# roseDwayane/EyeGaze-Multimodal

Hardware: AMD Instinct MI355X
Metric: train samples/sec (gaze+EEG windows) (higher is better)
Workload: dtype bf16; 1 GPU; cfg3: BASELINE configs[2]/[3]: + bidirectional cross-stream attention fusion; batch_per_gpu=256, global_batch=256, C=8, T=1024, seq_len=65, d_model=256, layers=6, step=fwd(train,dropout)+bwd+allreduce+clip+AdamW, parallelism=dp1

## Files before the change

### eyegaze_multimodal_amd/csrc/heads.hip

```cpp
#include "common.h"

namespace {

template <typename T>
__global__ void rows_bcast_f32_kernel(const float* __restrict__ src, const float* __restrict__ pos, T* __restrict__ dst,
                                      int NB, int S, int D, int R, int off, int src_nb) {
  const int b = blockIdx.y, r = blockIdx.x;
  const float* s = src + ((size_t)(b % src_nb) * R + r) * D;
  T* d = dst + ((size_t)b * S + off + r) * D;
  for (int n = threadIdx.x; n < D; n += blockDim.x) {
    float v = s[n];
    if (pos) v += pos[(size_t)(off + r) * D + n];
    Elem<T>::st(d + n, v);
  }
}

template <typename T>
__global__ void rows_copy_kernel(T* __restrict__ seq, int S, int D, int R, int off, int b_src0, int b_dst0) {
  const int b = blockIdx.y, r = blockIdx.x;
  const T* s = seq + ((size_t)(b_src0 + b) * S + off + r) * D;
  T* d = seq + ((size_t)(b_dst0 + b) * S + off + r) * D;
  for (int n = threadIdx.x; n < D; n += blockDim.x) d[n] = s[n];
}

// ... 480 lines not shown
          float g4[4];
          load4((const T*)&gv[u], g4);
#pragma unroll
          for (int e = 0; e < 4; ++e) v[e] = g4[e] > 0.f ? v[e] * gate_scale : 0.f;
          store4(dst + row_off(dmap, b * R + (s - off)) + n, v);
        }
      }
    }
  };
  for (int i = 0; i < iters; i += 8) rows8(r + 16 * i, 16, min(8, iters - i));
  if (j == 0) {
    const int b0 = bl + 16 * iters;
    if (b0 < NB) rows8(b0, 4, (NB - b0 + 3) / 4);
  }
#pragma unroll
  for (int e = 0; e < 4; ++e) red[r][tx * 4 + e] = acc[e];
  __syncthreads();
  if (threadIdx.x < 64) {
    const int c = threadIdx.x;
    float a[4];
#pragma unroll
    for (int l = 0; l < 4; ++l) a[l] = (red[l][c] + red[l + 4][c]) + (red[l + 8][c] + red[l + 12][c]);
    const float t = a[0] + a[1] + a[2] + a[3];
    const int col = blockIdx.y * 64 + c;
    out[(size_t)s * D + col] = t;
    if (s == 0 && cls_out) cls_out[col] = t;
  }
}

constexpr int HD = 256;
constexpr int HK = 3 * HD;
constexpr int HP = HD + 8;

template <typename T, int NT, int KS>
__device__ __forceinline__ void head_mma(f32x4 (&acc)[NT], const T* xrow, const T* __restrict__ W, const int ldw, const int n0,
                                         const int lane) {
  typedef typename H16<T>::frag frag;
  const int l15 = lane & 15, g = lane >> 4;
  const T* wp = W + (size_t)(n0 + l15) * ldw + 8 * g;
  frag wf[KS][NT];
#pragma unroll
  for (int ks = 0; ks < KS; ++ks)
#pragma unroll
    for (int t = 0; t < NT; ++t) wf[ks][t] = *(const frag*)(wp + (size_t)16 * t * ldw + 32 * ks);
  __builtin_amdgcn_sched_barrier(0);
#pragma unroll
  for (int ks = 0; ks < KS; ++ks) {
    const frag xf = *(const frag*)(xrow + 32 * ks);
#pragma unroll
    for (int t = 0; t < NT; ++t) acc[t] = H16<T>::mfma(wf[ks][t], xf, acc[t]);
  }
}

template <typename T>
struct HeadsFwd {
  const T* comb; T* zf; T* hcl; const T* Wsf; const T* Wc0;
  const float* bsf; const float* bc0; const float* W3; const float* b3;
  const long long* labels; float* logits; float* sloss; float* loss; unsigned int* counter;
  const eg_step_state* st;
  int B, ncls;
  DropCfg d1;
};

constexpr int HKP = HK + 8;
template <typename T>
__global__ __launch_bounds__(512) void heads_fwd_kernel(HeadsFwd<T> p) {
  __shared__ __attribute__((aligned(16))) T xs[2][16][HKP];
  __shared__ __attribute__((aligned(16))) T hs[16][HP];
  __shared__ float red[256];
  __shared__ int last_s;
  const int tid = threadIdx.x, lane = tid & 63, wave = tid >> 6;
  const int l15 = lane & 15, g = lane >> 4;
  const int m0 = blockIdx.x * 16;
  const int m = m0 + l15;
  const int n0 = 32 * wave;
  for (int c = tid; c < 16 * (HK / 8); c += 512) {
    const int r = c / (HK / 8), ch = c % (HK / 8);
    const size_t row = (size_t)min(m0 + r, p.B - 1) * HK;
    *(u32x4*)&xs[0][r][ch * 8] = *(const u32x4*)(p.comb + row + ch * 8);
    if (ch >= HD / 8) *(u32x4*)&xs[1][r][ch * 8] = *(const u32x4*)(p.zf + row + ch * 8);
  }
  __syncthreads();

  f32x4 acc[2];
#pragma unroll
  for (int t = 0; t < 2; ++t) acc[t] = (f32x4){0.f, 0.f, 0.f, 0.f};
  head_mma<T, 2, HK / 32>(acc, &xs[0][l15][8 * g], p.Wsf, HK, n0, lane);
#pragma unroll
  for (int t = 0; t < 2; ++t) {
    const int n = n0 + 16 * t + 4 * g;
    float bv[4], v[4];
    load4(p.bsf + n, bv);
#pragma unroll
    for (int e = 0; e < 4; ++e) v[e] = acc[t][e] + bv[e];
    store4(&xs[1][l15][n], v);
    if (m < p.B) store4(p.zf + (size_t)m * HK + n, v);
    acc[t] = (f32x4){0.f, 0.f, 0.f, 0.f};
  }
  __syncthreads();
  head_mma<T, 2, HK / 32>(acc, &xs[1][l15][8 * g], p.Wc0, HK, n0, lane);
  uint32_t seed_lo = 0, seed_hi = 0;
  if (p.d1.thresh) {
    seed_lo = p.st->seed_lo;
    seed_hi = p.st->seed_hi;
  }
#pragma unroll
  for (int t = 0; t < 2; ++t) {
    const int n = n0 + 16 * t + 4 * g;
    float bv[4], v[4];
    load4(p.bc0 + n, bv);
#pragma unroll
    for (int e = 0; e < 4; ++e) v[e] = fmaxf(acc[t][e] + bv[e], 0.f);
    eg_dropout_run<4>(v, p.d1, seed_lo, seed_hi, (uint32_t)m * (uint32_t)HD + (uint32_t)n);
    store4(&hs[l15][n], v);
    if (m < p.B) store4(p.hcl + (size_t)m * HD + n, v);
  }
  __syncthreads();
#pragma unroll
  for (int i = 0; i < 2; ++i) {
    const int r = 2 * wave + i;
    if (m0 + r < p.B)
      classifier_ce_fwd_row<T>(&hs[r][0], p.W3, p.b3, p.labels, p.logits, p.sloss, m0 + r, HD, p.ncls, lane);
  }
  if (!p.labels) return;
  __threadfence();
  __syncthreads();
  if (tid == 0) last_s = atomicAdd(p.counter, 1u) == gridDim.x - 1;
  __syncthreads();
  if (!last_s || tid >= 256) return;
  __threadfence();
  block_mean256<true>(p.sloss, p.loss, p.B, red);
  if (tid == 0) *p.counter = 0u;
}

constexpr int TNP = 128 + 8;
template <typename T>
__device__ __forceinline__ void small_tn_tile(const T* __restrict__ dY, const int ldy, const T* __restrict__ X, const int ldx,
                                              float* __restrict__ dW, float* __restrict__ db, const int M, const int K,
                                              const int tile, char* smem) {
  typedef typename H16<T>::frag frag;
  T (*Yt)[TNP] = (T(*)[TNP])smem;
  T (*Xt)[TNP] = (T(*)[TNP])(smem + 64 * TNP * sizeof(T));
  const int tid = threadIdx.x, lane = tid & 63, wave = tid >> 6;
  const int l15 = lane & 15, g = lane >> 4;
  const int tiles_k = K / 64;
  const int n0 = (tile / tiles_k) * 64, k0 = (tile % tiles_k) * 64;
  const int nsplit = M > 128 ? 2 : 1;
  const int kw = wave & 3, t0 = (wave >> 2) * 2, t1 = blockDim.x == 512 ? t0 + 2 : 4;
  f32x4 acc[2][4];
#pragma unroll
  for (int sp = 0; sp < 2; ++sp)
#pragma unroll
    for (int t = 0; t < 4; ++t) acc[sp][t] = (f32x4){0.f, 0.f, 0.f, 0.f};
  float bsplit[2] = {0.f, 0.f};
  for (int sp = 0; sp < nsplit; ++sp) {
    if (sp) __syncthreads();
    for (int c = tid; c < 1024; c += blockDim.x) {
      const int row = c >> 3, ch = c & 7;
      const int m = 128 * sp + row;
      u32x4 y = {0u, 0u, 0u, 0u}, x = {0u, 0u, 0u, 0u};
      if (m < M) {
        y = *(const u32x4*)(dY + (size_t)m * ldy + n0 + ch * 8);
        x = *(const u32x4*)(X + (size_t)m * ldx + k0 + ch * 8);
      }
      const uint16_t* ye = (const uint16_t*)&y;
// ... 10 lines not shown
      const frag xf = *(const frag*)&Xt[16 * kw + l15][32 * ks + 8 * g];
#pragma unroll
      for (int t = 0; t < 4; ++t)
        if (t >= t0 && t < t1) {
          const frag yf = *(const frag*)&Yt[16 * t + l15][32 * ks + 8 * g];
          acc[sp][t] = H16<T>::mfma(xf, yf, acc[sp][t]);
        }
    }
    if (db && k0 == 0 && tid < 64) {
      float bh[2] = {0.f, 0.f};
      for (int sub = 0; sub < 4; ++sub)
#pragma unroll
        for (int half = 0; half < 2; ++half) {
          float cs = 0.f;
#pragma unroll
          for (int i = 0; i < 16; ++i) cs += H16<T>::ld(Yt[tid][32 * sub + 16 * half + i]);
          bh[half] += cs;
        }
      bsplit[sp] = bh[0] + bh[1];
    }
  }
#pragma unroll
  for (int t = 0; t < 4; ++t)
    if (t >= t0 && t < t1) {
      const int n = n0 + 16 * t + l15, k = k0 + 16 * kw + 4 * g;
      f32x4 o = acc[0][t];
      if (nsplit == 2) o += acc[1][t];
      *(f32x4*)(dW + (size_t)n * K + k) = o;
    }
  if (db && k0 == 0 && tid < 64) db[n0 + tid] = nsplit == 2 ? bsplit[0] + bsplit[1] : bsplit[0];
}
constexpr int TN_SMEM = 2 * 64 * TNP * 2;

template <typename T>
__global__ __launch_bounds__(256) void classifier_ce_bwd_fused_kernel(const T* __restrict__ h, const float* __restrict__ W,
                                                                      const float* __restrict__ logits,
                                                                      const long long* __restrict__ labels,
                                                                      const float* __restrict__ gloss,
                                                                      const float* __restrict__ glogits,
                                                                      float* __restrict__ dlogits, T* __restrict__ dh,
                                                                      float* __restrict__ dW, float* __restrict__ db, int B,
                                                                      int K, int ncls, int use_gate, float gate_scale, int nce) {
  __shared__ __attribute__((aligned(16))) T hts[256][64];
  __shared__ float dls[256][16];
  __shared__ float red[4][64], redb[4];
  const int lane = threadIdx.x & 63, bl = threadIdx.x >> 6;
  if ((int)blockIdx.x < nce) {
    const int b = blockIdx.x * 4 + bl;
    if (b < B) classifier_ce_bwd_row<T>(b, lane, h, W, logits, labels, gloss, glogits, dlogits, dh, B, K, ncls, use_gate, gate_scale);
    return;
  }
  const int kb = (blockIdx.x - nce) * 64, k = kb + lane;
  const bool wide = kb + 64 <= K && K % 8 == 0;
  for (int c = threadIdx.x; c < B * 8; c += 256) {
    const int b = c >> 3, ch = c & 7;
    if (wide) *(u32x4*)&hts[b][ch * 8] = *(const u32x4*)(h + (size_t)b * K + kb + ch * 8);
    else
      for (int e = 0; e < 8; ++e)
        if (kb + ch * 8 + e < K) hts[b][ch * 8 + e] = h[(size_t)b * K + kb + ch * 8 + e];
  }
  for (int b = threadIdx.x; b < B; b += 256) {
    float dl[16];
    classifier_dlogits_row(logits, labels, gloss, glogits, b, B, ncls, dl);
#pragma unroll
    for (int c = 0; c < 16; ++c) dls[b][c] = dl[c];
  }
  __syncthreads();
  float s[16], sb[16];
#pragma unroll
  for (int c = 0; c < 16; ++c) s[c] = sb[c] = 0.f;
  for (int b = bl; b < B; b += 4) {
    const float hv = H16<T>::ld(hts[b][lane]);
#pragma unroll
    for (int c = 0; c < 16; ++c)
      if (c < ncls) {
        const float dl = dls[b][c];
        if (k < K) s[c] = fmaf(dl, hv, s[c]);
        sb[c] += dl;
      }
  }
#pragma unroll
  for (int c = 0; c < 16; ++c)
    if (c < ncls) {
      red[bl][lane] = s[c];
      if (lane == 0) redb[bl] = sb[c];
      __syncthreads();
      if (bl == 0) {
        if (k < K) dW[(size_t)c * K + k] = red[0][lane] + red[1][lane] + red[2][lane] + red[3][lane];
        if (kb == 0 && lane == 0) db[c] = redb[0] + redb[1] + redb[2] + redb[3];
      }
      __syncthreads();
    }
}

template <typename T>
__global__ __launch_bounds__(512) void heads_bwd_chain_kernel(const T* __restrict__ dhcl, const T* __restrict__ c0T,
                                                              const T* __restrict__ sfT, const T* __restrict__ zf,
                                                              T* __restrict__ dzf, T* __restrict__ dcomb, float* __restrict__ dWc0,
                                                              float* __restrict__ dbc0, int B, int nrt) {
  __shared__ __attribute__((aligned(16))) char smem[TN_SMEM];
  if ((int)blockIdx.x >= nrt) {
    small_tn_tile<T>(dhcl, HD, zf, HK, dWc0, dbc0, B, HK, blockIdx.x - nrt, smem);
    return;
  }
  T (*xs)[16][HP] = (T(*)[16][HP])smem;
  const int tid = threadIdx.x, lane = tid & 63, wave = tid >> 6;
  const int l15 = lane & 15, g = lane >> 4;
  const int m0 = blockIdx.x * 16;
  const int m = m0 + l15;
  {
    const int r = tid >> 5, ch = tid & 31;
    *(u32x4*)&xs[0][r][ch * 8] = *(const u32x4*)(dhcl + (size_t)min(m0 + r, B - 1) * HD + ch * 8);
  }
  __syncthreads();
#pragma unroll 1
  for (int prod = 0; prod < 2; ++prod) {
    const T* W = prod ? sfT : c0T;
    T* out = prod ? dcomb : dzf;
    const int n0 = 96 * wave;
    f32x4 acc[6];
#pragma unroll
    for (int t = 0; t < 6; ++t) acc[t] = (f32x4){0.f, 0.f, 0.f, 0.f};
    head_mma<T, 6, HD / 32>(acc, &xs[prod][l15][8 * g], W, HD, n0, lane);
#pragma unroll
    for (int t = 0; t < 6; ++t) {
      const int n = n0 + 16 * t + 4 * g;
      float v[4] = {acc[t][0] + 0.f, acc[t][1] + 0.f, acc[t][2] + 0.f, acc[t][3] + 0.f};
      if (!prod && n < HD) store4(&xs[1][l15][n], v);
      if (m < B) store4(out + (size_t)m * HK + n, v);
    }
    __syncthreads();
  }
}

template <typename T>
__global__ __launch_bounds__(256) void heads_bwd_pool_kernel(const T* __restrict__ z, const T* __restrict__ dcomb,
                                                             const T* __restrict__ dzf, const float* __restrict__ gcls1,
                                                             const float* __restrict__ gcls2, const T* __restrict__ dibs_pool,
                                                             const float* __restrict__ gibs_pool, T* __restrict__ dz,
                                                             const T* __restrict__ comb, float* __restrict__ dWsf,
                                                             float* __restrict__ dbsf, int B, int S, int D, int off, int n_ibs,
                                                             int ibs_first) {
  __shared__ __attribute__((aligned(16))) char smem[TN_SMEM];
  if ((int)blockIdx.x >= B) {
    small_tn_tile<T>(dzf, HK, comb, HK, dWsf, dbsf, B, HK, blockIdx.x - B, smem);
    return;
  }
  pool_fuse_bwd_sample<T>(blockIdx.x, z, dcomb, dzf, gcls1, gcls2, dibs_pool, gibs_pool, dz, B, S, D, off, n_ibs, ibs_first);
}

}

extern "C" int eg_rows_bcast_f32(const float* src, const float* pos, void* seq, int NB, int S, int D, int R, int off,
                                 int src_nb, int dtype, void* stream) {
  if (eg_dtype_check("eg_rows_bcast_f32", dtype, true)) return 1;
  EG_CHECK(src && seq && NB > 0 && R > 0 && off >= 0 && off + R <= S && src_nb > 0, "eg_rows_bcast_f32: bad arguments");
  dim3 grid(R, NB);
  hipStream_t s = (hipStream_t)stream;
  eg_dispatch_dtype(dtype, [&](auto t) {
    using T = typename decltype(t)::type;
    hipLaunchKernelGGL(rows_bcast_f32_kernel<T>, grid, dim3(256), 0, s, src, pos, (T*)seq, NB, S, D, R, off, src_nb);
  });
  EG_LAUNCH_CHECK("rows_bcast_f32");
  return 0;
}
// ... 109 lines not shown
  EG_LAUNCH_CHECK("rows_gather_gate");
  return 0;
}

extern "C" int eg_token_grad_tail(const void* dseq, const void* gate, void* dst, eg_rowmap dmap, float* pos_grad,
                                  float* cls_grad, int NB, int S, int D, int R, int off, float gate_scale, int dtype,
                                  void* stream) {
  if (eg_dtype_check("eg_token_grad_tail", dtype, false)) return 1;
  EG_CHECK(dseq && gate && dst && pos_grad, "eg_token_grad_tail: null pointer");
  EG_CHECK(NB > 0 && S > 0 && R > 0 && off >= 0 && off + R <= S, "eg_token_grad_tail: bad shape NB=%d S=%d R=%d off=%d", NB, S, R, off);
  EG_CHECK(D > 0 && D % 64 == 0, "eg_token_grad_tail: D=%d must be a multiple of 64", D);
  EG_CHECK(dmap.row_stride % 4 == 0 && dmap.group_stride % 4 == 0, "eg_token_grad_tail: destination rows must be 8-B aligned");
  hipStream_t s = (hipStream_t)stream;
  dim3 grid(S, D / 64);
  eg_dispatch_16(dtype, [&](auto t) {
    using T = typename decltype(t)::type;
    hipLaunchKernelGGL(token_grad_tail_kernel<T>, grid, dim3(256), 0, s, (const T*)dseq, (const T*)gate, (T*)dst, to_rowmap(dmap), pos_grad,
                       cls_grad, NB, S, D, R, off, gate_scale);
  });
  EG_LAUNCH_CHECK("token_grad_tail");
  return 0;
}

template <typename T>
static void launch_heads_fwd(const void* comb, void* zf, void* hcl, const void* Wsf, const float* bsf, const void* Wc0,
                             const float* bc0, const float* W3, const float* b3, const int64_t* labels, float* logits,
                             float* sloss, float* loss, uint32_t* counter, int B, int ncls, float drop_p, uint32_t drop_site,
                             const eg_step_state* state, hipStream_t s) {
  HeadsFwd<T> p;
  p.comb = (const T*)comb; p.zf = (T*)zf; p.hcl = (T*)hcl; p.Wsf = (const T*)Wsf; p.Wc0 = (const T*)Wc0;
  p.bsf = bsf; p.bc0 = bc0; p.W3 = W3; p.b3 = b3;
  p.labels = (const long long*)labels; p.logits = logits; p.sloss = sloss; p.loss = loss; p.counter = counter;
  p.st = state; p.B = B; p.ncls = ncls; p.d1 = make_drop(drop_p, drop_site);
  hipLaunchKernelGGL(heads_fwd_kernel<T>, dim3((B + 15) / 16), dim3(512), 0, s, p);
}

extern "C" int eg_heads_fwd(const void* comb, void* zf, void* hcl, const void* Wsf, const float* bsf, const void* Wc0,
                            const float* bc0, const float* W3, const float* b3, const int64_t* labels, float* logits,
                            float* sample_loss, float* loss, uint32_t* counter, int B, int D, int ncls, float drop_p,
                            uint32_t drop_site, const eg_step_state* state, int dtype, void* stream) {
  if (eg_dtype_check("eg_heads_fwd", dtype, false)) return 1;
  EG_CHECK(comb && zf && hcl && Wsf && bsf && Wc0 && bc0 && W3 && b3 && logits, "eg_heads_fwd: null pointer");
  EG_CHECK(D == HD, "eg_heads_fwd: d_model=%d (the fused heads are built for 256)", D);
  EG_CHECK(B > 0 && ncls > 0 && ncls <= 16, "eg_heads_fwd: B=%d, ncls=%d must be in [1,16]", B, ncls);
  EG_CHECK(!labels || (sample_loss && loss && counter), "eg_heads_fwd: labels need sample_loss, loss and the launch counter");
  EG_CHECK(drop_p >= 0.f && drop_p < 1.f && (drop_p == 0.f || state), "eg_heads_fwd: dropout needs the step state");
  EG_CHECK(((uintptr_t)comb | (uintptr_t)zf | (uintptr_t)hcl | (uintptr_t)Wsf | (uintptr_t)Wc0 | (uintptr_t)bsf | (uintptr_t)bc0) % 16 == 0,
           "eg_heads_fwd: alignment");
  hipStream_t s = (hipStream_t)stream;
  eg_dispatch_16(dtype, [&](auto t) {
    launch_heads_fwd<typename decltype(t)::type>(comb, zf, hcl, Wsf, bsf, Wc0, bc0, W3, b3, labels, logits, sample_loss, loss, counter, B,
                                                 ncls, drop_p, drop_site, state, s);
  });
  EG_LAUNCH_CHECK("heads_fwd");
  return 0;
}

extern "C" int eg_classifier_ce_bwd_fused(const void* h, const float* W, const float* logits, const int64_t* labels,
                                          const float* gloss, const float* glogits, float* dlogits, void* dh, float* dW,
                                          float* db, int B, int K, int ncls, int use_gate, float gate_scale, int dtype,
                                          void* stream) {
  if (eg_dtype_check("eg_classifier_ce_bwd_fused", dtype, false)) return 1;
  EG_CHECK(h && W && logits && dlogits && dh && dW && db, "eg_classifier_ce_bwd_fused: null pointer");
  EG_CHECK(B > 0 && B <= 256 && K > 0 && ncls > 0 && ncls <= 16, "eg_classifier_ce_bwd_fused: bad shape B=%d (<= 256) K=%d ncls=%d", B, K, ncls);
  EG_CHECK((uintptr_t)h % 16 == 0, "eg_classifier_ce_bwd_fused: alignment");
  hipStream_t s = (hipStream_t)stream;
  const int nce = (B + 3) / 4;
  dim3 grid(nce + (K + 63) / 64);
  eg_dispatch_16(dtype, [&](auto t) {
    using T = typename decltype(t)::type;
    hipLaunchKernelGGL(classifier_ce_bwd_fused_kernel<T>, grid, dim3(256), 0, s, (const T*)h, W, logits, (const long long*)labels, gloss,
                       glogits, dlogits, (T*)dh, dW, db, B, K, ncls, use_gate, gate_scale, nce);
  });
  EG_LAUNCH_CHECK("classifier_ce_bwd_fused");
  return 0;
}

extern "C" int eg_heads_bwd_chain(const void* dhcl, const void* c0T, const void* sfT, const void* zf, void* dzf, void* dcomb,
                                  float* dWc0, float* dbc0, int B, int D, int dtype, void* stream) {
  if (eg_dtype_check("eg_heads_bwd_chain", dtype, false)) return 1;
  EG_CHECK(dhcl && c0T && sfT && zf && dzf && dcomb && dWc0 && dbc0, "eg_heads_bwd_chain: null pointer");
  EG_CHECK(D == HD, "eg_heads_bwd_chain: d_model=%d (the fused heads are built for 256)", D);
  EG_CHECK(B > 0 && B <= 256, "eg_heads_bwd_chain: B=%d (the in-launch weight gradients sum at most 256 rows)", B);
  EG_CHECK(((uintptr_t)dhcl | (uintptr_t)c0T | (uintptr_t)sfT | (uintptr_t)zf | (uintptr_t)dzf | (uintptr_t)dcomb | (uintptr_t)dWc0) % 16 == 0,
           "eg_heads_bwd_chain: alignment");
  hipStream_t s = (hipStream_t)stream;
  const int nrt = (B + 15) / 16;
  dim3 grid(nrt + (HD / 64) * (HK / 64));
  eg_dispatch_16(dtype, [&](auto t) {
    using T = typename decltype(t)::type;
    hipLaunchKernelGGL(heads_bwd_chain_kernel<T>, grid, dim3(512), 0, s, (const T*)dhcl, (const T*)c0T, (const T*)sfT, (const T*)zf,
                       (T*)dzf, (T*)dcomb, dWc0, dbc0, B, nrt);
  });
  EG_LAUNCH_CHECK("heads_bwd_chain");
  return 0;
}

extern "C" int eg_heads_bwd_pool(const void* z, const void* dcomb, const void* dzf, const float* gcls1, const float* gcls2,
                                 const void* dibs_pool, const float* gibs_pool, void* dz, const void* comb, float* dWsf,
                                 float* dbsf, int B, int S, int D, int off, int n_ibs, int ibs_first, int dtype, void* stream) {
  if (eg_dtype_check("eg_heads_bwd_pool", dtype, false)) return 1;
  EG_CHECK(z && dcomb && dzf && dz && comb && dWsf && dbsf, "eg_heads_bwd_pool: null pointer");
  EG_CHECK(D == HD, "eg_heads_bwd_pool: d_model=%d (the fused heads are built for 256)", D);
  EG_CHECK(B > 0 && B <= 256 && off > 0 && off < S, "eg_heads_bwd_pool: bad shape B=%d (<= 256) S=%d off=%d", B, S, off);
  EG_CHECK(n_ibs == 0 || (ibs_first >= 1 && ibs_first + n_ibs <= S), "eg_heads_bwd_pool: ibs range");
  EG_CHECK(((uintptr_t)dzf | (uintptr_t)comb | (uintptr_t)dWsf) % 16 == 0, "eg_heads_bwd_pool: alignment");
  hipStream_t s = (hipStream_t)stream;
  dim3 grid(B + (HD / 64) * (HK / 64));
  eg_dispatch_16(dtype, [&](auto t) {
    using T = typename decltype(t)::type;
    hipLaunchKernelGGL(heads_bwd_pool_kernel<T>, grid, dim3(256), 0, s, (const T*)z, (const T*)dcomb, (const T*)dzf, gcls1, gcls2,
                       (const T*)dibs_pool, gibs_pool, (T*)dz, (const T*)comb, dWsf, dbsf, B, S, D, off, n_ibs, ibs_first);
  });
  EG_LAUNCH_CHECK("heads_bwd_pool");
  return 0;
}

__global__ __launch_bounds__(256) void fusion_loop_loss_kernel(const float* __restrict__ fused, const float* __restrict__ zi,
                                                               const float* __restrict__ ze, const long long* __restrict__ labels,
                                                               const float* __restrict__ prm, float* __restrict__ losses,
                                                               float* __restrict__ dfused, float* __restrict__ dai,
                                                               float* __restrict__ dae, float* __restrict__ dtau, int B, int K,
                                                               int mode, float eps_temp, float l_img, float l_eeg, float l_reg,
                                                               float t_min, float t_max, const eg_step_state* st) {
  __shared__ float red[3][256];
// ... 117 lines not shown
```

### eyegaze_multimodal_amd/engine.py

```python
from __future__ import annotations

import ctypes as C
import dataclasses
import math
import os
from collections import namedtuple
from typing import Dict, List, Optional, Tuple

import torch

from . import _lib as L
from . import tokens, wgrad_plan
from ._lib import EG_BF16, EG_F16, EG_F32, GemmDesc, GemmTNDesc, StepState, call, ptr, rowmap

SITE_CONV0, SITE_CONV1, SITE_SPEC, SITE_IBSTOK, SITE_IBSGEN, SITE_CLS, SITE_IBSCLS = 1, 2, 3, 4, 5, 6, 7
SITE_AUG_NOISE_R, SITE_AUG_NOISE_T, SITE_AUG_CHAN, SITE_AUG_TIME = 8, 9, 10, 11


@dataclasses.dataclass(frozen=True)
class WindowAugmentation:
    gaussian_noise_std: float = 0.0
    channel_dropout_prob: float = 0.0
    time_mask_max_length: int = 0
    time_mask_num: int = 0
# ... 482 lines not shown
        (_lay("sf", lambda d, F, e: (d, 3 * d), "cast", lambda d, F, e: (3 * d * d,), "symmetric_fusion.proj.weight"),),
        (_lay("sfT", lambda d, F, e: (3 * d, d), "transpose", lambda d, F, e: (d, 3 * d), "symmetric_fusion.proj.weight", bwd=True),),
        (_lay("c0", lambda d, F, e: (d, 3 * d), "cast", lambda d, F, e: (3 * d * d,), "classifier.0.weight"),),
        (_lay("c0T", lambda d, F, e: (3 * d, d), "transpose", lambda d, F, e: (d, 3 * d), "classifier.0.weight", bwd=True),)],
    "ibs": [
        (_lay("i0", lambda d, F, e: (d // 2, d), "cast", lambda d, F, e: ((d // 2) * d,), "ibs_classifier.0.weight"),),
        (_lay("i0T", lambda d, F, e: (d, _align(d // 2, e.bk)), "transpose", lambda d, F, e: (d // 2, d), "ibs_classifier.0.weight",
              bwd=True),)],
    "cnn": [
        (_lay("spc2", lambda d, F, e: (64, 384), "conv2d", lambda d, F, e: (64, 32, 0), "spec_conv.3.weight"),),
        (_lay("spc2T", lambda d, F, e: (32, 768), "conv2d", lambda d, F, e: (64, 32, 1), "spec_conv.3.weight", bwd=True),),
        (_lay("spp0", lambda d, F, e: (2 * d, 1024), "cast", lambda d, F, e: (2 * d * 1024,), "proj.0.weight"),),
        (_lay("spp0T", lambda d, F, e: (1024, 2 * d), "transpose", lambda d, F, e: (2 * d, 1024), "proj.0.weight", bwd=True),),
        (_lay("spp3", lambda d, F, e: (d, 2 * d), "cast", lambda d, F, e: (d * 2 * d,), "proj.3.weight"),),
        (_lay("spp3T", lambda d, F, e: (2 * d, d), "transpose", lambda d, F, e: (d, 2 * d), "proj.3.weight", bwd=True),)],
    "ibs_tok": [
        (_lay("ib0", lambda d, F, e: (64, e.C * e.C), "cast", lambda d, F, e: (64 * e.C * e.C,), "bottleneck.0.weight"),),
        (_lay("ib0T", lambda d, F, e: (e.C * e.C, 64), "transpose", lambda d, F, e: (64, e.C * e.C), "bottleneck.0.weight", bwd=True),),
        (_lay("ib3", lambda d, F, e: (d, 64), "cast", lambda d, F, e: (d * 64,), "bottleneck.3.weight"),),
        (_lay("ib3T", lambda d, F, e: (64, d), "transpose", lambda d, F, e: (d, 64), "bottleneck.3.weight", bwd=True),)],
    "ibs_gen": [
        (_lay("ig0", lambda d, F, e: (2 * d, 64), "conv", lambda d, F, e: (2 * d, 28, 1, 28, 64), "0.weight"),),
        (_lay("ig3", lambda d, F, e: (d, 2 * d), "cast", lambda d, F, e: (d * 2 * d,), "3.weight"),),
        (_lay("ig3T", lambda d, F, e: (2 * d, d), "transpose", lambda d, F, e: (d, 2 * d), "3.weight", bwd=True),)],
}
_ALL_LAYOUTS = [lay for groups in LAYOUTS.values() for group in groups for lay in group]
_FUSED_TWIN = {u.key: f for u in _ALL_LAYOUTS for f in _ALL_LAYOUTS
               if u.route and not (u.bwd or f.bwd or u.fused) and (f.route, f.src, f.fused) == (u.route, u.src, True)}


Rows = namedtuple("Rows", "qkv lse ctx r1 st1 y1 hff gbits r2 st2 out", defaults=(None,) * 11)


def _head_tensors(cfg, B: int):
    d, nc = cfg.d_model, cfg.num_classes
    t = {"cls1": ((B, d), True), "cls2": ((B, d), True), "comb": ((B, 3 * d), False), "zf": ((B, 3 * d), False), "hcl": ((B, d), False),
         "logits": ((B, nc), True), "sloss": ((B,), True), "loss": ((1,), True)}
    if cfg.use_ibs:
        t.update({"ibs_pool_f": ((B, d), True), "ibs_pool": ((B, d), False), "hib": ((B, d // 2), False),
                  "ibs_logits": ((B, nc), True), "ibs_sloss": ((B,), True), "ibs_loss": ((1,), True)})
    return t


class ForwardEngine(EngineBase):

    def __init__(self, model, B: int, T: int, device: torch.device, dtype: int, state_dev: Optional[torch.Tensor] = None):
        super().__init__(model, B, device, dtype)
        cfg = model.cfg
        self.cfg, self.T = cfg, T
        self.head_dim = attention_head_dim(cfg)
        if cfg.conv_layers != 2:
            raise L.EgError("HIP path implements the reference's 2-layer temporal conv front-end (conv_layers=2)")
        if cfg.d_model % 64 != 0 or cfg.d_ff % 64 != 0:
            raise L.EgError("d_model and d_ff must be multiples of 64")
        self.NB, self.C = 2 * B, cfg.in_channels
        self.geo = geometry(cfg, T, dtype)
        for name, v in self.geo._asdict().items():
            setattr(self, name, v)
        self.n_ibs = cfg.num_ibs_tokens
        self.n_spec = self.C if cfg.use_spectrogram else 0
        sequence_length(cfg, T)
        self.M = self.NB * self.S
        self._resolve_routes()
        self._alloc()
        tokens.alloc(self)
        self._init_state(state_dev)
# ... 6 lines not shown
        self._attn_core = "eg_attention_dk" if wide else "eg_attention_long" if self.attn_long else "eg_attention"
        self._attn_heads = (cfg.num_heads, self.head_dim) if wide else (cfg.num_heads,)
        self.attn_block = bool(env.get("EYEGAZE_ATTN_BLOCK", "1") != "0" and half
                               and L.lib().eg_attn_block_ok(self.S, cfg.d_model, cfg.num_heads, dtype))
        self.fuse_ffn = half and cfg.d_model == 256 and cfg.d_ff % 128 == 0
        self.ln_fuse = env.get("EYEGAZE_LN_FUSE", "1") != "0"
        self.fused_tail = half
        self.pack_unused = False

    def _reads(self, lay, l) -> bool:
        return lay.route is None or (bool(getattr(self, lay.route)) and l != "x") == lay.fused

    def _stages(self):
        yield "front", "", ""
        for l in range(self.cfg.num_layers):
            yield "attn", f"encoder.layers.{l}.mha.", l
            yield "ffn", f"encoder.layers.{l}.ffn.", l
        if self.cfg.use_cross_attention:
            yield "attn", "cross_attn.cross_attn.", "x"
        yield "heads", "", ""
        if self.cfg.use_ibs:
            yield "ibs", "", ""
        if self.cfg.use_spectrogram:
            yield "cnn", "spectrogram_generator.", ""
        if self.cfg.use_ibs:
            yield ("ibs_tok", "ibs_tokenizer.", "") if self.cfg.use_robust_ibs else ("ibs_gen", "ibs_generator.proj.", "")

    def _pack_body(self, record: bool):
        super()._pack_body(record)
        tokens.pack(self)

    def _head_alloc(self) -> Dict[str, torch.Tensor]:
        a = {n: self._t(*shape, dtype=(torch.float32 if is32 else None)) for n, (shape, is32) in _head_tensors(self.cfg, self.B).items()}
        a["heads_ctr"] = torch.zeros(1, device=self.device, dtype=torch.int32)
        return a

    def attn_unfused_fwd(self, x, l, kv_shift, sites, p, R: Rows):
        M, d = self.M, self.cfg.d_model
        pre, qkv, lse, ctx, r = _attn_prefix(l), R.qkv, R.lse, R.ctx, R.r1
        self.gemm(ptr(x), ptr(self.w[f"qkv{l}"]), ptr(qkv), M, 3 * d, d, bias=ptr(self.w[f"bqkv{l}"]))
        call(self._attn_core + "_fwd", ptr(qkv), ptr(ctx), ptr(lse), self.NB, self.S, *self._attn_heads,
             kv_shift, self.dtype, p, sites["attn"], self.st_ptr, self.stream)
        self._probs_hook(self.model.get_submodule(pre + "dropout"), qkv, lse, kv_shift)
        self._attn_stats(l, qkv, lse, kv_shift)
        self.gemm(ptr(ctx), ptr(self.w[f"o{l}"]), ptr(r), M, d, d, bias=self.fp.p_ptr(pre + "out_proj.bias"),
                  drop1=(p, sites["drop1"]), residual=ptr(x))

    def attn_block_fwd(self, x, l, p, sites, R: Rows, ln=None):
        w, fp, d = self.w, self.fp, self.cfg.d_model
        pre, qkv, lse, ctx, r1, lean = _attn_prefix(l), R.qkv, R.lse, R.ctx, R.r1, R.qkv is None
        dsc = L.AttnBlockDesc()
        dsc.x, dsc.wqkv_frag, dsc.wo_frag = ptr(x), ptr(w[f"wqkvb{l}"]), ptr(w[f"wob{l}"])
        dsc.bqkv, dsc.bo = ptr(w[f"bqkv{l}"]), fp.p_ptr(pre + "out_proj.bias")
        dsc.qkv, dsc.ctx, dsc.lse, dsc.r1 = ptr(qkv), ptr(ctx), ptr(lse), ptr(r1)
        dsc.state = self.st_ptr
        dsc.NB, dsc.S, dsc.d_model, dsc.num_heads, dsc.dtype = self.NB, self.S, d, self.cfg.num_heads, self.dtype
        dsc.attn_drop_p, dsc.attn_drop_site = p, sites["attn"]
        dsc.out_drop_p, dsc.out_drop_site = p, sites["drop1"]
        if ln is not None:
            dsc.ln_gamma, dsc.ln_beta = fp.p_ptr(ln[0] + ".weight"), fp.p_ptr(ln[0] + ".bias")
            dsc.ln_out, dsc.ln_stats = ptr(ln[1]), ptr(ln[2])

        def work():
            M, S, H = self.M, self.S, self.cfg.num_heads
            flops = 2.0 * M * d * 3 * d + 2.0 * M * d * d + 4.0 * self.NB * H * S * S * (d // H)
            nbytes = self.es * (M * d * 3 + M * 3 * d + 4 * d * d) + 4 * (self.NB * H * S + 4 * d)
            if ln is not None:
# ... 639 lines not shown
    a, sc = _inference_tensors(cfg, B, T, dtype)

    lean, scratch = (sum(math.prod(shape) * (4 if f32 else es) for shape, f32 in tab.values()) for tab in (a, sc))
    return lean + scratch, lean


class AttnStats:

    def __init__(self, where, map_sum: torch.Tensor, diag: torch.Tensor, scratch: torch.Tensor):
        self.stage = "x" if where == "cross" else int(where)
        self.map_sum, self.diag, self.scratch = map_sum, diag, scratch


class ConnStats:

    def __init__(self, labels: torch.Tensor, class_sum: torch.Tensor, class_count: torch.Tensor, scratch: torch.Tensor):
        self.labels, self.class_sum, self.class_count, self.scratch = labels, class_sum, class_count, scratch


class InferenceEngine(ForwardEngine):
    TRAINING_CALLS = ("backward", "accumulate", "optimizer_step", "set_state", "check_overflow_and_update_scaler")

    def _init_state(self, state_dev):
        self.state_dev = torch.zeros(L.STATE_WORDS, dtype=torch.int32, device=self.device)

    def _held(self, group, l, every: bool):
        return [lay if self._reads(lay, l) else _FUSED_TWIN[lay.key] for lay in group if not (lay.bwd or lay.fused)]

    def _alloc(self):
        self.w = self._alloc_w()
        shapes, self._sc_shapes = _inference_tensors(self.cfg, self.B, self.T, self.dtype)
        a = {n: self._t(*shape, dtype=(torch.float32 if is32 else None)) for n, (shape, is32) in shapes.items()}
        a["x0"] = a["xa"]
        a["heads_ctr"] = torch.zeros(1, device=self.device, dtype=torch.int32)
        self.a = a
        self.sc = {}
        self.routes_taken = []
        self.attn_stats: Optional[AttnStats] = None
        self.conn_stats: Optional[ConnStats] = None

    def _scratch(self, name: str) -> torch.Tensor:
        if name not in self.sc:
            shape, is32 = self._sc_shapes[name]
            self.sc[name] = self._t(*shape, dtype=(torch.float32 if is32 else None))
        return self.sc[name]

    def _rows(self, l, x) -> Rows:
        a, s = self.a, self._scratch
        out = a["xb"] if x is a["xa"] else a["xa"]
        if l == "norm":
            return Rows(st2=s("st"), out=out)
        if l == "x":
            return Rows(s("qkv"), s("lse"), s("ctx"), s("r"), s("st"), out=out)
        drop = self.model.encoder.layers[l].mha.dropout
        wanted = drop._forward_hooks or drop._forward_pre_hooks or (self.attn_stats is not None and self.attn_stats.stage == l)
        lean_attn = self.attn_block and self.ln_fuse and not wanted
        lean_ffn = self.fuse_ffn and self.ln_fuse
        self.routes_taken += [(l, "attn", "lean" if lean_attn else "scratch"), (l, "ffn", "lean" if lean_ffn else "scratch")]
        attn = (None,) * 5 if lean_attn else (s("qkv"), s("lse"), s("ctx"), s("r"), s("st"))
        ffn = (None,) * 4 if lean_ffn else (s("hff"), None, s("r"), s("st"))
        return Rows(*attn, a["y1"], *ffn, out)

    def _attn_stats(self, l, qkv, lse, kv_shift):
        st = self.attn_stats
        if st is None or st.stage != l:
            return
        for name, t, shape in (("map_sum", st.map_sum, (self.S, self.S)), ("diag", st.diag, (self.B, self.S))):
# ... 65 lines not shown
```

Baseline: 83790 samples/s.

## Split classifier head kernels into column-sliced launches for wider grid parallelism

```diff
diff --git a/eyegaze_multimodal_amd/csrc/heads.hip b/eyegaze_multimodal_amd/csrc/heads.hip
--- a/eyegaze_multimodal_amd/csrc/heads.hip
+++ b/eyegaze_multimodal_amd/csrc/heads.hip
@@ -536,25 +536,87 @@
 constexpr int HK = 3 * HD;
 constexpr int HP = HD + 8;
 
-template <typename T, int NT, int KS>
-__device__ __forceinline__ void head_mma(f32x4 (&acc)[NT], const T* xrow, const T* __restrict__ W, const int ldw, const int n0,
-                                         const int lane) {
+template <typename T, int KS>
+__device__ __forceinline__ f32x4 slice_mma(const T* __restrict__ xrow, const T* __restrict__ wrow) {
   typedef typename H16<T>::frag frag;
-  const int l15 = lane & 15, g = lane >> 4;
-  const T* wp = W + (size_t)(n0 + l15) * ldw + 8 * g;
-  frag wf[KS][NT];
-#pragma unroll
-  for (int ks = 0; ks < KS; ++ks)
-#pragma unroll
-    for (int t = 0; t < NT; ++t) wf[ks][t] = *(const frag*)(wp + (size_t)16 * t * ldw + 32 * ks);
+  frag wf[KS], xf[KS];
+#pragma unroll
+  for (int ks = 0; ks < KS; ++ks) wf[ks] = *(const frag*)(wrow + 32 * ks);
+#pragma unroll
+  for (int ks = 0; ks < KS; ++ks) xf[ks] = *(const frag*)(xrow + 32 * ks);
   __builtin_amdgcn_sched_barrier(0);
-#pragma unroll
-  for (int ks = 0; ks < KS; ++ks) {
-    const frag xf = *(const frag*)(xrow + 32 * ks);
-#pragma unroll
-    for (int t = 0; t < NT; ++t) acc[t] = H16<T>::mfma(wf[ks][t], xf, acc[t]);
-  }
-}
+  f32x4 acc = (f32x4){0.f, 0.f, 0.f, 0.f};
+#pragma unroll
+  for (int ks = 0; ks < KS; ++ks) acc = H16<T>::mfma(wf[ks], xf[ks], acc);
+  return acc;
+}
+
+template <typename T, int R, int NC>
+__device__ __forceinline__ void classifier_ce_fwd_rows(const T* hs, const int pitch, const float* __restrict__ W,
+                                                       const float* __restrict__ bias, const long long* __restrict__ labels,
+                                                       float* __restrict__ logits, float* __restrict__ sample_loss, const int b0,
+                                                       const int nrows, const int ncls, const int lane) {
+  float w[NC][HD / 64], bs[NC], lg[R][NC];
+  int y[R];
+#pragma unroll
+  for (int c = 0; c < NC; ++c) {
+    const int cc = min(c, ncls - 1);
+#pragma unroll
+    for (int i = 0; i < HD / 64; ++i) w[c][i] = W[(size_t)cc * HD + lane + 64 * i];
+    bs[c] = bias[cc];
+  }
+#pragma unroll
+  for (int r = 0; r < R; ++r) {
+    y[r] = (labels && sample_loss && r < nrows) ? (int)labels[b0 + r] : -1;
+#pragma unroll
+    for (int c = 0; c < NC; ++c) lg[r][c] = 0.f;
+  }
+#pragma unroll
+  for (int i = 0; i < HD / 64; ++i)
+#pragma unroll
+    for (int r = 0; r < R; ++r) {
+      const float x = Elem<T>::ld(hs + (size_t)r * pitch + lane + 64 * i);
+#pragma unroll
+      for (int c = 0; c < NC; ++c) lg[r][c] += x * w[c][i];
+    }
+#pragma unroll
+  for (int r = 0; r < R; ++r)
+#pragma unroll
+    for (int c = 0; c < NC; ++c) lg[r][c] = wave_sum(lg[r][c]) + bs[c];
+  if (lane != 0) return;
+#pragma unroll
+  for (int r = 0; r < R; ++r) {
+    if (r >= nrows) break;
+    const int b = b0 + r;
+    float mx = -INFINITY, se = 0.f, ly = 0.f;
+#pragma unroll
+    for (int c = 0; c < NC; ++c)
+      if (c < ncls) mx = fmaxf(mx, lg[r][c]);
+#pragma unroll
+    for (int c = 0; c < NC; ++c)
+      if (c < ncls) {
+        logits[(size_t)b * ncls + c] = lg[r][c];
+        se += expf(lg[r][c] - mx);
+        if (c == y[r]) ly = lg[r][c];
+      }
+    if (labels && sample_loss) sample_loss[b] = (mx + logf(se)) - ly;
+  }
+}
+
+__device__ __forceinline__ bool last_arrival(unsigned int* ctr, const int total, int* flag) {
+  __syncthreads();
+  if (threadIdx.x == 0) {
+    __builtin_amdgcn_fence(__ATOMIC_RELEASE, "agent");
+    const bool last = atomicAdd(ctr, 1u) == (unsigned)(total - 1);
+    __builtin_amdgcn_fence(__ATOMIC_ACQUIRE, "agent");
+    if (last) *ctr = 0u;
+    *flag = last;
+  }
+  __syncthreads();
+  return *flag != 0;
+}
+
+constexpr int HSL = 64;
 
 template <typename T>
 struct HeadsFwd {
@@ -566,75 +628,64 @@
   DropCfg d1;
 };
 
-constexpr int HKP = HK + 8;
-template <typename T>
-__global__ __launch_bounds__(512) void heads_fwd_kernel(HeadsFwd<T> p) {
-  __shared__ __attribute__((aligned(16))) T xs[2][16][HKP];
+template <typename T>
+__global__ __launch_bounds__(256) void heads_fwd_sf_kernel(HeadsFwd<T> p) {
+  const int lane = threadIdx.x & 63, wave = threadIdx.x >> 6;
+  const int l15 = lane & 15, g = lane >> 4;
+  const int m = (blockIdx.x / (HD / HSL)) * 16 + l15;
+  const int n0 = (blockIdx.x % (HD / HSL)) * HSL + 16 * wave;
+  const f32x4 acc = slice_mma<T, HK / 32>(p.comb + (size_t)min(m, p.B - 1) * HK + 8 * g, p.Wsf + (size_t)(n0 + l15) * HK + 8 * g);
+  const int n = n0 + 4 * g;
+  float bv[4], v[4];
+  load4(p.bsf + n, bv);
+#pragma unroll
+  for (int e = 0; e < 4; ++e) v[e] = acc[e] + bv[e];
+  if (m < p.B) store4(p.zf + (size_t)m * HK + n, v);
+}
+
+template <typename T>
+__global__ __launch_bounds__(256) void heads_fwd_cls_kernel(HeadsFwd<T> p) {
   __shared__ __attribute__((aligned(16))) T hs[16][HP];
   __shared__ float red[256];
   __shared__ int last_s;
   const int tid = threadIdx.x, lane = tid & 63, wave = tid >> 6;
   const int l15 = lane & 15, g = lane >> 4;
-  const int m0 = blockIdx.x * 16;
-  const int m = m0 + l15;
-  const int n0 = 32 * wave;
-  for (int c = tid; c < 16 * (HK / 8); c += 512) {
-    const int r = c / (HK / 8), ch = c % (HK / 8);
-    const size_t row = (size_t)min(m0 + r, p.B - 1) * HK;
-    *(u32x4*)&xs[0][r][ch * 8] = *(const u32x4*)(p.comb + row + ch * 8);
-    if (ch >= HD / 8) *(u32x4*)&xs[1][r][ch * 8] = *(const u32x4*)(p.zf + row + ch * 8);
-  }
-  __syncthreads();
-
-  f32x4 acc[2];
-#pragma unroll
-  for (int t = 0; t < 2; ++t) acc[t] = (f32x4){0.f, 0.f, 0.f, 0.f};
-  head_mma<T, 2, HK / 32>(acc, &xs[0][l15][8 * g], p.Wsf, HK, n0, lane);
-#pragma unroll
-  for (int t = 0; t < 2; ++t) {
-    const int n = n0 + 16 * t + 4 * g;
-    float bv[4], v[4];
-    load4(p.bsf + n, bv);
-#pragma unroll
-    for (int e = 0; e < 4; ++e) v[e] = acc[t][e] + bv[e];
-    store4(&xs[1][l15][n], v);
-    if (m < p.B) store4(p.zf + (size_t)m * HK + n, v);
-    acc[t] = (f32x4){0.f, 0.f, 0.f, 0.f};
-  }
-  __syncthreads();
-  head_mma<T, 2, HK / 32>(acc, &xs[1][l15][8 * g], p.Wc0, HK, n0, lane);
+  const int grp = blockIdx.x / (HD / HSL), ngrp = gridDim.x / (HD / HSL);
+  const int m0 = grp * 16, m = m0 + l15;
+  const int n0 = (blockIdx.x % (HD / HSL)) * HSL + 16 * wave;
+  const f32x4 acc = slice_mma<T, HK / 32>(p.zf + (size_t)min(m, p.B - 1) * HK + 8 * g, p.Wc0 + (size_t)(n0 + l15) * HK + 8 * g);
   uint32_t seed_lo = 0, seed_hi = 0;
   if (p.d1.thresh) {
     seed_lo = p.st->seed_lo;
     seed_hi = p.st->seed_hi;
   }
-#pragma unroll
-  for (int t = 0; t < 2; ++t) {
-    const int n = n0 + 16 * t + 4 * g;
+  {
+    const int n = n0 + 4 * g;
     float bv[4], v[4];
     load4(p.bc0 + n, bv);
 #pragma unroll
-    for (int e = 0; e < 4; ++e) v[e] = fmaxf(acc[t][e] + bv[e], 0.f);
+    for (int e = 0; e < 4; ++e) v[e] = fmaxf(acc[e] + bv[e], 0.f);
     eg_dropout_run<4>(v, p.d1, seed_lo, seed_hi, (uint32_t)m * (uint32_t)HD + (uint32_t)n);
-    store4(&hs[l15][n], v);
     if (m < p.B) store4(p.hcl + (size_t)m * HD + n, v);
   }
+  if (!last_arrival(p.counter + 1 + grp, HD / HSL, &last_s)) return;
+  for (int c = tid; c < 16 * (HD / 4); c += 256) {
+    const int r = c / (HD / 4), ch = c % (HD / 4);
+    const T* src = p.hcl + (size_t)min(m0 + r, p.B - 1) * HD + ch * 4;
+    *(unsigned long long*)&hs[r][ch * 4] = __hip_atomic_load((const unsigned long long*)src, __ATOMIC_RELAXED, __HIP_MEMORY_SCOPE_AGENT);
+  }
   __syncthreads();
-#pragma unroll
-  for (int i = 0; i < 2; ++i) {
-    const int r = 2 * wave + i;
-    if (m0 + r < p.B)
-      classifier_ce_fwd_row<T>(&hs[r][0], p.W3, p.b3, p.labels, p.logits, p.sloss, m0 + r, HD, p.ncls, lane);
-  }
-  if (!p.labels) return;
-  __threadfence();
-  __syncthreads();
-  if (tid == 0) last_s = atomicAdd(p.counter, 1u) == gridDim.x - 1;
-  __syncthreads();
-  if (!last_s || tid >= 256) return;
-  __threadfence();
+  {
+    const int b0 = m0 + 4 * wave, nrows = min(4, p.B - b0);
+    if (nrows > 0) {
+      if (p.ncls <= 4)
+        classifier_ce_fwd_rows<T, 4, 4>(&hs[4 * wave][0], HP, p.W3, p.b3, p.labels, p.logits, p.sloss, b0, nrows, p.ncls, lane);
+      else
+        classifier_ce_fwd_rows<T, 4, 16>(&hs[4 * wave][0], HP, p.W3, p.b3, p.labels, p.logits, p.sloss, b0, nrows, p.ncls, lane);
+    }
+  }
+  if (!p.labels || !last_arrival(p.counter, ngrp, &last_s)) return;
   block_mean256<true>(p.sloss, p.loss, p.B, red);
-  if (tid == 0) *p.counter = 0u;
 }
 
 constexpr int TNP = 128 + 8;
@@ -711,6 +762,128 @@
 }
 constexpr int TN_SMEM = 2 * 64 * TNP * 2;
 
+template <int NC>
+__device__ __forceinline__ void classifier_dlogits_row_pre(const float* __restrict__ logits, const long long* __restrict__ labels,
+                                                           const float* __restrict__ gloss, const float* __restrict__ glogits,
+                                                           const int b, int B, int ncls, float (&dl)[NC]) {
+  float lg[NC], ge[NC];
+#pragma unroll
+  for (int c = 0; c < NC; ++c) {
+    const int cc = min(c, ncls - 1);
+    lg[c] = logits[(size_t)b * ncls + cc];
+    ge[c] = glogits ? glogits[(size_t)b * ncls + cc] : 0.f;
+  }
+  const float gl = (gloss && labels) ? *gloss / (float)B : 0.f;
+  const int y = labels ? (int)labels[b] : -1;
+  float mx = -INFINITY;
+#pragma unroll
+  for (int c = 0; c < NC; ++c)
+    if (c < ncls) mx = fmaxf(mx, lg[c]);
+  float se = 0.f;
+#pragma unroll
+  for (int c = 0; c < NC; ++c) {
+    dl[c] = 0.f;
+    if (c < ncls) {
+      dl[c] = expf(lg[c] - mx);
+      se += dl[c];
+    }
+  }
+#pragma unroll
+  for (int c = 0; c < NC; ++c)
+    if (c < ncls) {
+#pragma clang fp contract(off)
+      float d = gl * (dl[c] / se - (c == y ? 1.f : 0.f));
+      if (glogits) d += ge[c];
+      dl[c] = d;
+    }
+}
+
+template <typename T, int NC>
+__device__ __forceinline__ void classifier_ce_bwd_fused_body(const T* __restrict__ h, const float* __restrict__ W,
+                                                             const float* __restrict__ logits, const long long* __restrict__ labels,
+                                                             const float* __restrict__ gloss, const float* __restrict__ glogits,
+                                                             float* __restrict__ dlogits, T* __restrict__ dh, float* __restrict__ dW,
+                                                             float* __restrict__ db, int B, int K, int ncls, int use_gate,
+                                                             float gate_scale, int nce, T (*hts)[64], float (*dls)[16],
+                                                             float (*red)[64], float* redb) {
+  const int lane = threadIdx.x & 63, bl = threadIdx.x >> 6;
+  if ((int)blockIdx.x < nce) {
+    const int b = blockIdx.x * 4 + bl;
+    if (b >= B) return;
+    float dl[NC];
+    classifier_dlogits_row_pre<NC>(logits, labels, gloss, glogits, b, B, ncls, dl);
+    if (lane == 0) {
+#pragma unroll
+      for (int c = 0; c < NC; ++c)
+        if (c < ncls) dlogits[(size_t)b * ncls + c] = dl[c];
+    }
+    for (int k0 = lane; k0 < K; k0 += 256) {
+      float w[4][NC], hv[4];
+#pragma unroll
+      for (int j = 0; j < 4; ++j) {
+        const int kk = min(k0 + 64 * j, K - 1);
+#pragma unroll
+        for (int c = 0; c < NC; ++c) w[j][c] = W[(size_t)min(c, ncls - 1) * K + kk];
+        hv[j] = use_gate ? Elem<T>::ld(h + (size_t)b * K + kk) : 1.f;
+      }
+#pragma unroll
+      for (int j = 0; j < 4; ++j) {
+        float s = 0.f;
+#pragma unroll
+        for (int c = 0; c < NC; ++c)
+          if (c < ncls) s += dl[c] * w[j][c];
+        if (use_gate) s = hv[j] > 0.f ? s * gate_scale : 0.f;
+        if (k0 + 64 * j < K) Elem<T>::st(dh + (size_t)b * K + k0 + 64 * j, s);
+      }
+    }
+    return;
+  }
+  const int kb = (blockIdx.x - nce) * 64, k = kb + lane;
+  const bool wide = kb + 64 <= K && K % 8 == 0;
+  for (int c = threadIdx.x; c < B * 8; c += 256) {
+    const int b = c >> 3, ch = c & 7;
+    if (wide) *(u32x4*)&hts[b][ch * 8] = *(const u32x4*)(h + (size_t)b * K + kb + ch * 8);
+    else
+      for (int e = 0; e < 8; ++e)
+        if (kb + ch * 8 + e < K) hts[b][ch * 8 + e] = h[(size_t)b * K + kb + ch * 8 + e];
+  }
+  for (int b = threadIdx.x; b < B; b += 256) {
+    float dl[NC];
+    classifier_dlogits_row_pre<NC>(logits, labels, gloss, glogits, b, B, ncls, dl);
+#pragma unroll
+    for (int c = 0; c < NC; ++c) dls[b][c] = dl[c];
+  }
+  __syncthreads();
+  float s[NC], sb[NC];
+#pragma unroll
+  for (int c = 0; c < NC; ++c) s[c] = sb[c] = 0.f;
+#pragma unroll 8
+  for (int b = bl; b < B; b += 4) {
+    const float hv = H16<T>::ld(hts[b][lane]);
+#pragma unroll
+    for (int c4 = 0; c4 < NC; c4 += 4) {
+      const f32x4 d4 = *(const f32x4*)&dls[b][c4];
+#pragma unroll
+      for (int e = 0; e < 4; ++e) {
+        if (k < K) s[c4 + e] = fmaf(d4[e], hv, s[c4 + e]);
+        sb[c4 + e] += d4[e];
+      }
+    }
+  }
+#pragma unroll
+  for (int c = 0; c < NC; ++c)
+    if (c < ncls) {
+      red[bl][lane] = s[c];
+      if (lane == 0) redb[bl] = sb[c];
+      __syncthreads();
+      if (bl == 0) {
+        if (k < K) dW[(size_t)c * K + k] = red[0][lane] + red[1][lane] + red[2][lane] + red[3][lane];
+        if (kb == 0 && lane == 0) db[c] = redb[0] + redb[1] + redb[2] + redb[3];
+      }
+      __syncthreads();
+    }
+}
+
 template <typename T>
 __global__ __launch_bounds__(256) void classifier_ce_bwd_fused_kernel(const T* __restrict__ h, const float* __restrict__ W,
                                                                       const float* __restrict__ logits,
@@ -721,95 +894,44 @@
                                                                       float* __restrict__ dW, float* __restrict__ db, int B,
                                                                       int K, int ncls, int use_gate, float gate_scale, int nce) {
   __shared__ __attribute__((aligned(16))) T hts[256][64];
-  __shared__ float dls[256][16];
+  __shared__ __attribute__((aligned(16))) float dls[256][16];
   __shared__ float red[4][64], redb[4];
-  const int lane = threadIdx.x & 63, bl = threadIdx.x >> 6;
-  if ((int)blockIdx.x < nce) {
-    const int b = blockIdx.x * 4 + bl;
-    if (b < B) classifier_ce_bwd_row<T>(b, lane, h, W, logits, labels, gloss, glogits, dlogits, dh, B, K, ncls, use_gate, gate_scale);
+  if (ncls <= 4)
+    classifier_ce_bwd_fused_body<T, 4>(h, W, logits, labels, gloss, glogits, dlogits, dh, dW, db, B, K, ncls, use_gate, gate_scale, nce,
+                                       hts, dls, red, redb);
+  else
+    classifier_ce_bwd_fused_body<T, 16>(h, W, logits, labels, gloss, glogits, dlogits, dh, dW, db, B, K, ncls, use_gate, gate_scale, nce,
+                                        hts, dls, red, redb);
+}
+
+template <typename T>
+__global__ __launch_bounds__(256) void heads_bwd_dzf_kernel(const T* __restrict__ dhcl, const T* __restrict__ c0T,
+                                                            const T* __restrict__ zf, T* __restrict__ dzf,
+                                                            float* __restrict__ dWc0, float* __restrict__ dbc0, int B, int nsl) {
+  __shared__ __attribute__((aligned(16))) char smem[TN_SMEM];
+  if ((int)blockIdx.x >= nsl) {
+    small_tn_tile<T>(dhcl, HD, zf, HK, dWc0, dbc0, B, HK, blockIdx.x - nsl, smem);
     return;
   }
-  const int kb = (blockIdx.x - nce) * 64, k = kb + lane;
-  const bool wide = kb + 64 <= K && K % 8 == 0;
-  for (int c = threadIdx.x; c < B * 8; c += 256) {
-    const int b = c >> 3, ch = c & 7;
-    if (wide) *(u32x4*)&hts[b][ch * 8] = *(const u32x4*)(h + (size_t)b * K + kb + ch * 8);
-    else
-      for (int e = 0; e < 8; ++e)
-        if (kb + ch * 8 + e < K) hts[b][ch * 8 + e] = h[(size_t)b * K + kb + ch * 8 + e];
-  }
-  for (int b = threadIdx.x; b < B; b += 256) {
-    float dl[16];
-    classifier_dlogits_row(logits, labels, gloss, glogits, b, B, ncls, dl);
-#pragma unroll
-    for (int c = 0; c < 16; ++c) dls[b][c] = dl[c];
-  }
-  __syncthreads();
-  float s[16], sb[16];
-#pragma unroll
-  for (int c = 0; c < 16; ++c) s[c] = sb[c] = 0.f;
-  for (int b = bl; b < B; b += 4) {
-    const float hv = H16<T>::ld(hts[b][lane]);
-#pragma unroll
-    for (int c = 0; c < 16; ++c)
-      if (c < ncls) {
-        const float dl = dls[b][c];
-        if (k < K) s[c] = fmaf(dl, hv, s[c]);
-        sb[c] += dl;
-      }
-  }
-#pragma unroll
-  for (int c = 0; c < 16; ++c)
-    if (c < ncls) {
-      red[bl][lane] = s[c];
-      if (lane == 0) redb[bl] = sb[c];
-      __syncthreads();
-      if (bl == 0) {
-        if (k < K) dW[(size_t)c * K + k] = red[0][lane] + red[1][lane] + red[2][lane] + red[3][lane];
-        if (kb == 0 && lane == 0) db[c] = redb[0] + redb[1] + redb[2] + redb[3];
-      }
-      __syncthreads();
-    }
-}
-
-template <typename T>
-__global__ __launch_bounds__(512) void heads_bwd_chain_kernel(const T* __restrict__ dhcl, const T* __restrict__ c0T,
-                                                              const T* __restrict__ sfT, const T* __restrict__ zf,
-                                                              T* __restrict__ dzf, T* __restrict__ dcomb, float* __restrict__ dWc0,
-                                                              float* __restrict__ dbc0, int B, int nrt) {
-  __shared__ __attribute__((aligned(16))) char smem[TN_SMEM];
-  if ((int)blockIdx.x >= nrt) {
-    small_tn_tile<T>(dhcl, HD, zf, HK, dWc0, dbc0, B, HK, blockIdx.x - nrt, smem);
-    return;
-  }
-  T (*xs)[16][HP] = (T(*)[16][HP])smem;
-  const int tid = threadIdx.x, lane = tid & 63, wave = tid >> 6;
+  const int lane = threadIdx.x & 63, wave = threadIdx.x >> 6;
   const int l15 = lane & 15, g = lane >> 4;
-  const int m0 = blockIdx.x * 16;
-  const int m = m0 + l15;
-  {
-    const int r = tid >> 5, ch = tid & 31;
-    *(u32x4*)&xs[0][r][ch * 8] = *(const u32x4*)(dhcl + (size_t)min(m0 + r, B - 1) * HD + ch * 8);
-  }
-  __syncthreads();
-#pragma unroll 1
-  for (int prod = 0; prod < 2; ++prod) {
-    const T* W = prod ? sfT : c0T;
-    T* out = prod ? dcomb : dzf;
-    const int n0 = 96 * wave;
-    f32x4 acc[6];
-#pragma unroll
-    for (int t = 0; t < 6; ++t) acc[t] = (f32x4){0.f, 0.f, 0.f, 0.f};
-    head_mma<T, 6, HD / 32>(acc, &xs[prod][l15][8 * g], W, HD, n0, lane);
-#pragma unroll
-    for (int t = 0; t < 6; ++t) {
-      const int n = n0 + 16 * t + 4 * g;
-      float v[4] = {acc[t][0] + 0.f, acc[t][1] + 0.f, acc[t][2] + 0.f, acc[t][3] + 0.f};
-      if (!prod && n < HD) store4(&xs[1][l15][n], v);
-      if (m < B) store4(out + (size_t)m * HK + n, v);
-    }
-    __syncthreads();
-  }
+  const int m = (blockIdx.x / (HK / HSL)) * 16 + l15;
+  const int n0 = (blockIdx.x % (HK / HSL)) * HSL + 16 * wave;
+  const f32x4 acc = slice_mma<T, HD / 32>(dhcl + (size_t)min(m, B - 1) * HD + 8 * g, c0T + (size_t)(n0 + l15) * HD + 8 * g);
+  const float v[4] = {acc[0] + 0.f, acc[1] + 0.f, acc[2] + 0.f, acc[3] + 0.f};
+  if (m < B) store4(dzf + (size_t)m * HK + n0 + 4 * g, v);
+}
+
+template <typename T>
+__global__ __launch_bounds__(256) void heads_bwd_dcomb_kernel(const T* __restrict__ dzf, const T* __restrict__ sfT,
+                                                              T* __restrict__ dcomb, int B) {
+  const int lane = threadIdx.x & 63, wave = threadIdx.x >> 6;
+  const int l15 = lane & 15, g = lane >> 4;
+  const int m = (blockIdx.x / (HK / HSL)) * 16 + l15;
+  const int n0 = (blockIdx.x % (HK / HSL)) * HSL + 16 * wave;
+  const f32x4 acc = slice_mma<T, HD / 32>(dzf + (size_t)min(m, B - 1) * HK + 8 * g, sfT + (size_t)(n0 + l15) * HD + 8 * g);
+  const float v[4] = {acc[0] + 0.f, acc[1] + 0.f, acc[2] + 0.f, acc[3] + 0.f};
+  if (m < B) store4(dcomb + (size_t)m * HK + n0 + 4 * g, v);
 }
 
 template <typename T>
@@ -985,7 +1107,9 @@
   p.bsf = bsf; p.bc0 = bc0; p.W3 = W3; p.b3 = b3;
   p.labels = (const long long*)labels; p.logits = logits; p.sloss = sloss; p.loss = loss; p.counter = counter;
   p.st = state; p.B = B; p.ncls = ncls; p.d1 = make_drop(drop_p, drop_site);
-  hipLaunchKernelGGL(heads_fwd_kernel<T>, dim3((B + 15) / 16), dim3(512), 0, s, p);
+  const dim3 grid(((B + 15) / 16) * (HD / HSL));
+  hipLaunchKernelGGL(heads_fwd_sf_kernel<T>, grid, dim3(256), 0, s, p);
+  hipLaunchKernelGGL(heads_fwd_cls_kernel<T>, grid, dim3(256), 0, s, p);
 }
 
 extern "C" int eg_heads_fwd(const void* comb, void* zf, void* hcl, const void* Wsf, const float* bsf, const void* Wc0,
@@ -1000,6 +1124,7 @@
   EG_CHECK(drop_p >= 0.f && drop_p < 1.f && (drop_p == 0.f || state), "eg_heads_fwd: dropout needs the step state");
   EG_CHECK(((uintptr_t)comb | (uintptr_t)zf | (uintptr_t)hcl | (uintptr_t)Wsf | (uintptr_t)Wc0 | (uintptr_t)bsf | (uintptr_t)bc0) % 16 == 0,
            "eg_heads_fwd: alignment");
+  EG_CHECK(counter, "eg_heads_fwd: the launch counters (1 + ceil(B / 16) zeroed words) are needed with and without labels");
   hipStream_t s = (hipStream_t)stream;
   eg_dispatch_16(dtype, [&](auto t) {
     launch_heads_fwd<typename decltype(t)::type>(comb, zf, hcl, Wsf, bsf, Wc0, bc0, W3, b3, labels, logits, sample_loss, loss, counter, B,
@@ -1038,12 +1163,12 @@
   EG_CHECK(((uintptr_t)dhcl | (uintptr_t)c0T | (uintptr_t)sfT | (uintptr_t)zf | (uintptr_t)dzf | (uintptr_t)dcomb | (uintptr_t)dWc0) % 16 == 0,
            "eg_heads_bwd_chain: alignment");
   hipStream_t s = (hipStream_t)stream;
-  const int nrt = (B + 15) / 16;
-  dim3 grid(nrt + (HD / 64) * (HK / 64));
+  const int nsl = ((B + 15) / 16) * (HK / HSL);
   eg_dispatch_16(dtype, [&](auto t) {
     using T = typename decltype(t)::type;
-    hipLaunchKernelGGL(heads_bwd_chain_kernel<T>, grid, dim3(512), 0, s, (const T*)dhcl, (const T*)c0T, (const T*)sfT, (const T*)zf,
-                       (T*)dzf, (T*)dcomb, dWc0, dbc0, B, nrt);
+    hipLaunchKernelGGL(heads_bwd_dzf_kernel<T>, dim3(nsl + (HD / 64) * (HK / 64)), dim3(256), 0, s, (const T*)dhcl, (const T*)c0T,
+                       (const T*)zf, (T*)dzf, dWc0, dbc0, B, nsl);
+    hipLaunchKernelGGL(heads_bwd_dcomb_kernel<T>, dim3(nsl), dim3(256), 0, s, (const T*)dzf, (const T*)sfT, (T*)dcomb, B);
   });
   EG_LAUNCH_CHECK("heads_bwd_chain");
   return 0;
diff --git a/eyegaze_multimodal_amd/engine.py b/eyegaze_multimodal_amd/engine.py
--- a/eyegaze_multimodal_amd/engine.py
+++ b/eyegaze_multimodal_amd/engine.py
@@ -538,6 +538,10 @@
 Rows = namedtuple("Rows", "qkv lse ctx r1 st1 y1 hff gbits r2 st2 out", defaults=(None,) * 11)
 
 
+def _heads_counters(B: int, device) -> torch.Tensor:
+    return torch.zeros(1 + (B + 15) // 16, device=device, dtype=torch.int32)
+
+
 def _head_tensors(cfg, B: int):
     d, nc = cfg.d_model, cfg.num_classes
     t = {"cls1": ((B, d), True), "cls2": ((B, d), True), "comb": ((B, 3 * d), False), "zf": ((B, 3 * d), False), "hcl": ((B, d), False),
@@ -610,7 +614,7 @@
 
     def _head_alloc(self) -> Dict[str, torch.Tensor]:
         a = {n: self._t(*shape, dtype=(torch.float32 if is32 else None)) for n, (shape, is32) in _head_tensors(self.cfg, self.B).items()}
-        a["heads_ctr"] = torch.zeros(1, device=self.device, dtype=torch.int32)
+        a["heads_ctr"] = _heads_counters(self.B, self.device)
         return a
 
     def attn_unfused_fwd(self, x, l, kv_shift, sites, p, R: Rows):
@@ -1316,7 +1320,7 @@
         shapes, self._sc_shapes = _inference_tensors(self.cfg, self.B, self.T, self.dtype)
         a = {n: self._t(*shape, dtype=(torch.float32 if is32 else None)) for n, (shape, is32) in shapes.items()}
         a["x0"] = a["xa"]
-        a["heads_ctr"] = torch.zeros(1, device=self.device, dtype=torch.int32)
+        a["heads_ctr"] = _heads_counters(self.B, self.device)
         self.a = a
         self.sc = {}
         self.routes_taken = []
```

New measurement: 85180 samples/s (median of 6 runs). +1.7%, better.
